# JavierMtz5/robotic_manipulator_rloa

Measured on AMD Instinct MI355X. Metric: env-steps/s (= learn() updates/s at update_freq=1,num_updates=1), KUKA 6-DoF NAF batch=256, higher is better.
Workload: dtype f32; 1 GPU; configs[1]: kuka shapes S=21 A=6 H=256, 64 envs/GPU, batch 256, HBM replay 1000000, HIP NAF head (hadamard P), 64 learn() per vector step; launch=hipGraph, parallelism=single, chain=rows, fused_kernels=bb,ep,gb,hk,s2, grad_exchange=none

## Files before the change

### include/naf_hip.h

```cpp
#ifndef NAF_HIP_H
#define NAF_HIP_H

#include <stddef.h>
#include <stdint.h>

#ifdef __cplusplus
extern "C" {
#endif

#define NAF_OK 0
#define NAF_ERR_ARG (-1)
#define NAF_ERR_STATE (-2)

#define NAF_P_HADAMARD 0
#define NAF_P_MATMUL 1

#define NAF_ACTION_TRUNC_INT 0
#define NAF_ACTION_FLOAT 1

typedef struct naf_replay naf_replay_t;

#define NAF_XGMI_MAX_WORLD 8
#define NAF_XGMI_HANDLE_BYTES 64
typedef struct {
// ... 11 lines not shown
int naf_timeline_read(int kernel_id, long long* out);

int naf_host_store_supported(int device);
int naf_host_publish(void* dst_device, const void* src_host, size_t bytes);
int naf_host_publish_launch(void* dst_device, const void* src_host, size_t bytes, void* graph_exec, void* stream);
int naf_host_store_alloc(size_t bytes, void** out_device_ptr);
int naf_host_store_free(void* device_ptr);
int naf_host_store_selftest(void* dst_device, int n_patterns, void* stream);

int naf_replay_row_floats(int S, int A);
int naf_replay_row_off_next_state(int S, int A);
int naf_replay_create(uint64_t capacity, int S, int A, float* rows, uint64_t* meta, naf_replay_t** out);
int naf_replay_destroy(naf_replay_t* h);
int naf_replay_size(naf_replay_t* h, uint64_t* size_out , void* stream);
int naf_replay_add_batch(naf_replay_t* h, const float* src_rows, int n, void* stream);
int naf_replay_add_counted(naf_replay_t* h, const float* src_rows, const int32_t* n_word, int n_max, void* stream);
int naf_replay_sample_indices(naf_replay_t* h, uint64_t seed, const uint64_t* counter_dev, uint64_t counter_off,
                              int32_t* idx, int B, int n_batches, int without_replacement, void* stream);
int naf_replay_sample_scratch_ints(int B);
int naf_replay_sample_indices_big(naf_replay_t* h, uint64_t seed, const uint64_t* counter_dev, uint64_t counter_off, int32_t* idx,
                                  int B, int n_batches, int without_replacement, int32_t* scratch, void* stream);
int naf_replay_batch_row_floats(int S, int A);
int naf_replay_gather_rows(naf_replay_t* h, const int32_t* idx, float* out_rows, int n, int out_ld, int action_mode,
                           void* stream);
int naf_replay_gather_soa(naf_replay_t* h, const int32_t* idx, float* s, float* u, float* r, float* s2,
                          float* d, int n, int action_mode, void* stream);
int naf_counter_add(uint64_t* p, uint64_t inc, void* stream);

int naf_head_fwd(const float* heads_pre, int ldh, const float* u, int ldu, float* q, float* mu_out ,
                 int B, int A, int p_mode, void* stream);
// ... 164 lines not shown
int naf_adam_polyak_fused(float* theta, const float* g, float* m, float* v, float* theta_target,
                          const float* partials, int n_partials, float max_norm, float lr, float beta1, float beta2,
                          float eps, float tau, float one_minus_tau, const int32_t* step_dev, float inv_world, size_t n,
                          void* stream);
int naf_polyak_update(float* target, const float* main, float tau, float one_minus_tau, size_t n, void* stream);

#define NAF_STEP_SPEC_INTS 12
typedef struct naf_step_copies {
    const void* src[3];
    void* dst[3];
    int n_words[3];
} naf_step_copies_t;
int naf_step_prep(naf_replay_t* h, const float* src_row, const int32_t* n_word, float* row_out, uint64_t seed,
                  uint64_t* counter_dev, int32_t* idx_out, float* out_rows, int out_ld, int action_mode, float* mom, int B,
                  int without_replacement, int32_t* spec_rec, const int32_t* idx_spec, const naf_step_copies_t* copies, void* stream);
typedef struct naf_step_prefetch {
    naf_replay_t* replay;
    uint64_t seed;
    uint64_t* counter_dev;
    int32_t* idx_spec;
    float* out_rows;
    int out_ld, action_mode;
    float* mom;
    int B, without_replacement;
    int32_t* spec_rec;
    int mode;
    const float* src_row;
    const int32_t* n_word;
    float* row_out;
    int32_t* idx_out;
// ... 40 lines not shown
                               uint64_t* host_errors, uint32_t* host_seq, uint32_t* action_rec, const naf_step_prefetch_t* prefetch,
                               int obs_system_scope, const naf_bb_layer1_t* layer1, void* stream);

typedef struct naf_episode_record {
    double score;
    int32_t frames;
    int32_t done;
    float last_reward;
    int32_t episode;
    uint32_t step_lo;
    uint32_t env;
} naf_episode_record_t;
int naf_synth_env_step(float* env_state, const float* actions, float* out_rows, float* obs_next, int E, int A,
                       uint64_t seed, const uint64_t* counter_dev, int max_frames, naf_episode_record_t* records,
                       int record_slots, void* stream);
#define NAF_SYNTH_PRESET_FLOATS 23
int naf_synth_env_reset(float* env_state, float* obs, int E, int A, uint64_t seed, uint64_t counter,
                        const float* preset_host, int preset_floats, void* stream);
int naf_synth_env_state_floats(int A);

#define NAF_CHAIN_BLOB_VERSION 1
#define NAF_CHAIN_HEADER_FLOATS 16
#define NAF_CHAIN_JOINT_FLOATS 24
#define NAF_CHAIN_SEGMENT_FLOATS 8
#define NAF_CHAIN_SCENE_FLOATS 8
#define NAF_CHAIN_ERR_VERSION (-11)
#define NAF_CHAIN_ERR_SIZE (-12)
#define NAF_CHAIN_ERR_COUNTS (-13)
#define NAF_CHAIN_ERR_VALUE (-14)
#define NAF_CHAIN_ERR_EE (-15)
// ... 61 lines not shown
```

### robotic_manipulator_rloa_amd/_lib.py

```python
from __future__ import annotations

import ctypes as C
import os
import re
import shutil
import subprocess
from typing import Optional

CSRC = os.path.join(os.path.dirname(os.path.abspath(__file__)), "csrc")
LIB_PATH = os.path.join(CSRC, "libnaf_hip.so")
SOURCES = ["lib.hip", "replay.hip", "naf_head.hip", "bn_relu.hip", "fused_layers.hip", "big_batch.hip", "gemm_bundle.hip", "optim.hip",
           "synth_env.hip", "xgmi_reduce.hip", "policy_act.hip", "step_path.hip", "naf_head_wide.hip",
           "state_digest.hip", "chain_env.hip"]
HEADERS = ["common.h", "head_body.h", "bn_tile.h", "xgmi_dev.h", "adam_body.h", "bn2bwd_fold.h", "act_body.h", "moments_body.h", "sample_body.h", "replay_dev.h", os.path.join("..", "..", "include", "naf_hip.h")]

P_HADAMARD, P_MATMUL = 0, 1
ACTION_TRUNC_INT, ACTION_FLOAT = 0, 1
NORM_CHUNK = 4096


class NafHipError(RuntimeError):
    pass


# ... 117 lines not shown
_vp, _i, _f, _u64, _sz, _i64 = C.c_void_p, C.c_int, C.c_float, C.c_uint64, C.c_size_t, C.c_int64

_PROTOS = {
    "naf_hip_abi_version": [],
    "naf_hip_arch": [],
    "naf_timeline_read": [_i, _vp],
    "naf_host_store_supported": [_i],
    "naf_host_publish": [_vp, _vp, _sz],
    "naf_host_publish_launch": [_vp, _vp, _sz, _vp, _vp],
    "naf_replay_row_floats": [_i, _i],
    "naf_replay_row_off_next_state": [_i, _i],
    "naf_replay_create": [_u64, _i, _i, _vp, _vp, C.POINTER(_vp)],
    "naf_replay_destroy": [_vp],
    "naf_replay_size": [_vp, C.POINTER(_u64), _vp],
    "naf_replay_add_batch": [_vp, _vp, _i, _vp],
    "naf_replay_add_counted": [_vp, _vp, _vp, _i, _vp],
    "naf_replay_sample_indices": [_vp, _u64, _vp, _u64, _vp, _i, _i, _i, _vp],
    "naf_replay_sample_scratch_ints": [_i],
    "naf_replay_sample_indices_big": [_vp, _u64, _vp, _u64, _vp, _i, _i, _i, _vp, _vp],
    "naf_replay_batch_row_floats": [_i, _i],
    "naf_replay_gather_rows": [_vp, _vp, _vp, _i, _i, _i, _vp],
    "naf_replay_gather_soa": [_vp, _vp, _vp, _vp, _vp, _vp, _vp, _i, _i, _vp],
    "naf_counter_add": [_vp, _u64, _vp],
    "naf_head_fwd": [_vp, _i, _vp, _i, _vp, _vp, _i, _i, _i, _vp],
    "naf_head_bwd": [_vp, _i, _vp, _i, _vp, _vp, _i, _i, _i, _vp],
    "naf_head_fwd_bwd_mse": [_vp, _i, _vp, _i, _vp, _i, _vp, _i, _f, _vp, _vp, _vp, _i, _i, _i, _vp],
    "naf_head_fwd_bwd_mse_splitk": [_vp, _i64, _vp, _i, _i, _vp, _i, _vp, _i, _f, _vp, _vp, _vp, _i, _i, _i, _vp],
    "naf_act_noise": [_vp, _i, _vp, _u64, _vp, _u64, _f, _i, _i, _i, _vp],
    "naf_bn_relu_fwd_train": [_vp, _i64, _i, _vp, _vp, _vp, _i64, _vp, _vp, _i64, _vp, _i64, _i, _vp, _vp, _i, _i, _i,
                              _f, _f, _vp],
# ... 15 lines not shown
                           _f, _f, _vp, _vp],
    "naf_bb_linear_stats_adam": [_vp, _i64, _i, _vp, _vp, _i64, _vp, _i64, _i, _vp, _i, _i, _i, _i, _vp, _vp],
    "naf_bb_layer2_head_rows": [_i],
    "naf_bb_layer2_head_exchange_floats": [_i, _i],
    "naf_bb_layer2_head": [_vp, _i64, _i, _vp, _vp, _i64, _vp, _vp, _vp, _i64, _vp, _i, _vp, _vp, _vp, _i64, _i, _i, _vp, _i, _vp,
                           _i, _f, _vp, _vp, _vp, _vp, _i, _vp, _i, _i, _i, _i, _f, _f, _vp, _vp],
    "naf_bb_layer1_bwd_kp": [_i],
    "naf_bb_layer1_bwd_finish_blocks": [_i],
    "naf_bb_layer1_bwd_finish": [_vp, _i, _vp, _i, _vp, _i, _vp, _vp, _vp, _vp, _vp, _vp, _vp, _vp, _vp, _vp, _vp, _vp, _vp, _i, _i,
                                 _vp, _i, _vp, _vp, _vp, _sz, _vp],
    "naf_gemm_bundle": [_vp, _i, _vp],
    "naf_grad_norm_partials": [_vp, _sz, _vp, _vp, _vp],
    "naf_adam_polyak_fused": [_vp, _vp, _vp, _vp, _vp, _vp, _i, _f, _f, _f, _f, _f, _f, _f, _vp, _f, _sz, _vp],
    "naf_polyak_update": [_vp, _vp, _f, _f, _sz, _vp],
    "naf_synth_env_step": [_vp, _vp, _vp, _vp, _i, _i, _u64, _vp, _i, _vp, _i, _vp],
    "naf_synth_env_reset": [_vp, _vp, _i, _i, _u64, _u64, _vp, _i, _vp],
    "naf_synth_env_state_floats": [_i],
    "naf_policy_act": [_vp, _i, _i, _vp, _vp, _vp, _vp, _vp, _vp, _vp, _vp, _vp, _i, _i, _vp, _vp, _vp, _vp, _f, _i, _vp, _i,
                       _vp, _u64, _vp, _vp, _f, _i, _i, _i, _vp],
    "naf_step_prep": [_vp, _vp, _vp, _vp, _u64, _vp, _vp, _vp, _i, _i, _vp, _i, _i, _vp, _vp, _vp, _vp],
    "naf_adam_polyak_act_sync_ints": [],
    "naf_host_store_alloc": [_sz, C.POINTER(_vp)],
    "naf_host_store_free": [_vp],
    "naf_host_store_selftest": [_vp, _i, _vp],
    "naf_step_prefetch": [_vp, _vp],
    "naf_step_launch": [_vp, _vp, _sz, _vp, _vp, _vp, _vp, C.c_int],
    "naf_adam_polyak_act": [_vp, _vp, _vp, _vp, _vp, _u64, _vp, _f, _i, _vp, _vp, _vp, _vp, _vp, _i, _vp],
    "naf_adam_polyak_act_layer1": [_vp, _vp, _vp, _vp, _vp, _u64, _vp, _f, _i, _vp, _vp, _vp, _vp, _vp, _i, _vp, _vp],
    "naf_xgmi_chunk_floats": [],
    "naf_xgmi_create": [_i, _i, _sz, C.c_double, C.POINTER(_vp)],
    "naf_xgmi_set_timeout": [_vp, C.c_double],
    "naf_xgmi_mem_kind": [_vp],
    "naf_xgmi_export": [_vp, _vp],
    "naf_xgmi_connect": [_vp, _vp, _vp],
    "naf_xgmi_connect_local": [_vp, _vp],
# ... 152 lines not shown
```

### robotic_manipulator_rloa_amd/csrc/replay.hip

```cpp
#include <stdlib.h>
#include "common.h"
#include "sample_body.h"
#include "replay_dev.h"
#include "../../include/naf_hip.h"
#include <new>

extern "C" int naf_replay_row_floats(int S, int A) {
    if (S <= 0 || A <= 0) return NAF_ERR_ARG;
    int need = naf_row_off_done(S, A) + 1;
    int rf = 32;
    while (rf < need) rf *= 2;
    return rf;
}

extern "C" int naf_replay_row_off_next_state(int S, int A) {
    if (S <= 0 || A <= 0) return NAF_ERR_ARG;
    return naf_row_off_s2(S, A);
}

extern "C" int naf_replay_create(uint64_t capacity, int S, int A, float* rows, uint64_t* meta, naf_replay_t** out) {
    if (!out || !rows || !meta || capacity == 0 || S <= 0 || A <= 0 || A > NAF_MAX_A_WIDE) return NAF_ERR_ARG;
    if (capacity > 0x7fffffffull) return NAF_ERR_ARG;
    if (((uintptr_t)rows & 15) != 0) return NAF_ERR_ARG;
    naf_replay* h = new (std::nothrow) naf_replay;
// ... 25 lines not shown
}

__global__ void replay_add_rows_kernel(float4* __restrict__ ring, const uint64_t* __restrict__ meta,
                                       const float4* __restrict__ src, int n, uint64_t cap, int rf4_shift) {
    const uint64_t head = meta[META_HEAD];
    const int rf4 = 1 << rf4_shift;
    for (int64_t g = (int64_t)blockIdx.x * blockDim.x + threadIdx.x; g < ((int64_t)n << rf4_shift);
         g += (int64_t)gridDim.x * blockDim.x) {
        int64_t r = g >> rf4_shift;
        int c = (int)(g & (rf4 - 1));
        uint64_t phys = (head + (uint64_t)r) % cap;
        ring[(phys << rf4_shift) + c] = src[g];
    }
}

__global__ void replay_advance_kernel(uint64_t* meta, uint64_t n, uint64_t cap) {
    if (blockIdx.x == 0 && threadIdx.x == 0) {
        uint64_t head = meta[META_HEAD], size = meta[META_SIZE];
        meta[META_HEAD] = (head + n) % cap;
        size += n;
        meta[META_SIZE] = size > cap ? cap : size;
        meta[META_TOTAL] += n;
    }
}

__global__ __launch_bounds__(1024) void replay_add_small_kernel(float4* __restrict__ ring, uint64_t* meta,
                                                                const float4* __restrict__ src, int n,
                                                                uint64_t cap, int rf4_shift) {
    const uint64_t head = meta[META_HEAD];
    const uint64_t size = meta[META_SIZE];
    const int rf4 = 1 << rf4_shift;
    __syncthreads();
    int g = threadIdx.x;
    if (g < (n << rf4_shift)) {
        int r = g >> rf4_shift;
        int c = g & (rf4 - 1);
        uint64_t phys = (head + (uint64_t)r) % cap;
        ring[(phys << rf4_shift) + c] = src[g];
    }
    if (threadIdx.x == 0) {
        meta[META_HEAD] = (head + (uint64_t)n) % cap;
        uint64_t s2 = size + (uint64_t)n;
        meta[META_SIZE] = s2 > cap ? cap : s2;
        meta[META_TOTAL] += (uint64_t)n;
    }
}

__global__ __launch_bounds__(1024) void replay_add_counted_kernel(float4* __restrict__ ring, uint64_t* meta,
                                                                  const float4* __restrict__ src, const int32_t* n_word,
                                                                  int n_max, uint64_t cap, int rf4_shift) {
    int n = __builtin_nontemporal_load(n_word);
    n = n < 0 ? 0 : (n > n_max ? n_max : n);
    const uint64_t head = meta[META_HEAD];
    const uint64_t size = meta[META_SIZE];
    const int rf4 = 1 << rf4_shift;
    __syncthreads();
    int g = threadIdx.x;
    if (g < (n << rf4_shift)) {
        int r = g >> rf4_shift;
// ... 3 lines not shown
    }
    if (threadIdx.x == 0 && n > 0) {
        meta[META_HEAD] = (head + (uint64_t)n) % cap;
        uint64_t s2 = size + (uint64_t)n;
        meta[META_SIZE] = s2 > cap ? cap : s2;
        meta[META_TOTAL] += (uint64_t)n;
    }
}

static inline int ilog2_exact(int x) {
    int s = 0;
    while ((1 << s) < x) ++s;
    return s;
}

extern "C" int naf_replay_add_batch(naf_replay_t* h, const float* src_rows, int n, void* stream) {
    if (!h || h->magic != NAF_REPLAY_MAGIC) return NAF_ERR_STATE;
    if (!src_rows || n < 0 || (uint64_t)n > h->capacity || ((uintptr_t)src_rows & 15) != 0) return NAF_ERR_ARG;
    if (n == 0) return NAF_OK;
    hipStream_t st = (hipStream_t)stream;
    const int rf4 = h->row_floats / 4;
    const int sh = ilog2_exact(rf4);
    if ((int64_t)n * rf4 <= 1024) {
        int threads = naf_round_up(n * rf4, 64);
        replay_add_small_kernel<<<1, threads, 0, st>>>((float4*)h->rows, h->meta, (const float4*)src_rows, n,
                                                        h->capacity, sh);
        NAF_CHECK_LAUNCH();
        return NAF_OK;
    }
    int64_t total = (int64_t)n * rf4;
    int blocks = (int)((total + 255) / 256);
    if (blocks > 4096) blocks = 4096;
    replay_add_rows_kernel<<<blocks, 256, 0, st>>>((float4*)h->rows, h->meta, (const float4*)src_rows, n,
                                                    h->capacity, sh);
    NAF_CHECK_LAUNCH();
    replay_advance_kernel<<<1, 64, 0, st>>>(h->meta, (uint64_t)n, h->capacity);
    NAF_CHECK_LAUNCH();
    return NAF_OK;
}

extern "C" int naf_replay_add_counted(naf_replay_t* h, const float* src_rows, const int32_t* n_word, int n_max, void* stream) {
    if (!h || h->magic != NAF_REPLAY_MAGIC) return NAF_ERR_STATE;
    const int rf4 = h->row_floats / 4;
    if (!src_rows || !n_word || n_max < 1 || (uint64_t)n_max > h->capacity || (int64_t)n_max * rf4 > 1024 ||
        ((uintptr_t)src_rows & 15) != 0 || ((uintptr_t)n_word & 3) != 0)
        return NAF_ERR_ARG;
    replay_add_counted_kernel<<<1, naf_round_up(n_max * rf4, 64), 0, (hipStream_t)stream>>>(
        (float4*)h->rows, h->meta, (const float4*)src_rows, n_word, n_max, h->capacity, ilog2_exact(rf4));
    NAF_CHECK_LAUNCH();
    return NAF_OK;
}

__global__ __launch_bounds__(1024) void replay_sample_kernel(const uint64_t* __restrict__ meta, uint64_t seed,
// ... 312 lines not shown
```

### robotic_manipulator_rloa_amd/csrc/replay_dev.h

```cpp
#pragma once
#include "common.h"
#include "../../include/naf_hip.h"

struct naf_replay {
    uint64_t capacity;
    int S, A, row_floats;
    float* rows;
    uint64_t* meta;
    uint32_t magic;
};
#define NAF_REPLAY_MAGIC 0x4e414652u

enum { META_HEAD = 0, META_SIZE = 1, META_TOTAL = 2, META_SAMPLE_CTR = 3, META_BAD_IDX = 7 };
```

### robotic_manipulator_rloa_amd/csrc/step_path.hip

```cpp
#include <string.h>
#include "common.h"
#include "../../include/naf_hip.h"
NAF_TL_DECL(g_tl_sp);
#ifdef NAF_TIMELINE
#define BM_MARK(slot) NAF_TL(g_tl_sp, NAF_TL_STEP_PREP, slot)
#define SB_MARK(slot) NAF_TL(g_tl_sp, NAF_TL_STEP_PREP, slot)
#endif
#include "act_body.h"
#include "adam_body.h"
#include "head_body.h"
#ifdef NAF_TIMELINE
#define BB_L1_TL(slot, is_first, is_last) NAF_TL_FL(g_tl_sp, NAF_TL_BB_LAYER1, slot, is_first, is_last)
#define BB_L1_TL_T(slot, is_first, is_last, thread) NAF_TL_FL_T(g_tl_sp, NAF_TL_BB_LAYER1, slot, is_first, is_last, thread)
#endif
#include "layer1_body.h"
#include "moments_body.h"
#include "replay_dev.h"
#include "sample_body.h"

NAF_TL_READER(naf_tl_read_sp, g_tl_sp)

#define SP_THREADS 1024
#define SP_RPT 4
#define SP_CACHE_ROWS 256
// ... 392 lines not shown
        for (const void* k : ks) {
            hipError_t e = hipFuncSetAttribute(k, hipFuncAttributeMaxDynamicSharedMemorySize, SP_MAX_DYN_LDS);
            if (e != hipSuccess) return (int)e;
        }
        raised_dev[dev] = 1;
    }
    const bool cache = sp_cached(B, out_ld);
    if (k4 <= 6 && cache) step_prep_kernel<6, true><<<1, SP_THREADS, lds, (hipStream_t)stream>>>(P);
    else if (k4 <= 6) step_prep_kernel<6, false><<<1, SP_THREADS, lds, (hipStream_t)stream>>>(P);
    else if (cache) step_prep_kernel<8, true><<<1, SP_THREADS, lds, (hipStream_t)stream>>>(P);
    else step_prep_kernel<8, false><<<1, SP_THREADS, lds, (hipStream_t)stream>>>(P);
    NAF_CHECK_LAUNCH();
    return NAF_OK;
}

#define AA_THREADS 512
#define AA_H 256
#define AA_L1_WGS 8
#define AA_L1_ROWS (AA_H / AA_L1_WGS)
#define AA_L2_WGS 32
#define AA_SYNC_RIDE (16 + 4 * 2 * AA_H)
#define AA_POLL_TICKS 200000LL

typedef float aa_f4 __attribute__((ext_vector_type(4)));

struct AdamActArgs {
    AdamArgs ad;
    int64_t off_W1, off_b1, off_g1, off_be1, off_W2, off_b2, off_g2, off_be2, off_Wh;
    int S, NH, NHP, HP, A;
    const float* obs;
// ... 745 lines not shown
```

### robotic_manipulator_rloa_amd/csrc/synth_env.hip

```cpp
#include "common.h"
#include "../../include/naf_hip.h"

#define ENV_STATE_FLOATS 36
#define ENV_OFF_VAR 24
#define ENV_OFF_SCORE 32
#define ENV_DT (1.0f / 240.0f)

struct EnvCfg {
    float link[8];
};
__constant__ EnvCfg c_env = {{0.34f, 0.02f, 0.40f, 0.02f, 0.40f, 0.13f, 0.05f, 0.05f}};

__device__ static inline void fk_chain(const float* q, int A, float* ee, const float* obstacle, float obstacle_r,
                                       bool* hit) {
    float R[9] = {1, 0, 0, 0, 1, 0, 0, 0, 1};
    float p[3] = {0.f, 0.f, 0.f};
    bool h = false;
    for (int k = 0; k < A; ++k) {
        float c = cosf(q[k]), s = sinf(q[k]);
        float N[9];
        if ((k & 1) == 0) {
            for (int r = 0; r < 3; ++r) {
                N[r * 3 + 0] = R[r * 3 + 0] * c + R[r * 3 + 1] * s;
                N[r * 3 + 1] = -R[r * 3 + 0] * s + R[r * 3 + 1] * c;
// ... 45 lines not shown
    for (int k = 0; k < 8; ++k) { st[14 + k] = preset.v[k]; st[ENV_OFF_VAR + k] = preset.v[15 + k]; }
    st[34] = st[35] = 0.f;
    for (int k = 0; k < 3; ++k) { st[8 + k] = preset.v[8 + k]; st[11 + k] = preset.v[11 + k]; }
    if (preset.v[14] > 0.f) {
        Philox4 p = philox4x32_10((uint32_t)seed, (uint32_t)(seed >> 32), (uint32_t)e, 0x4f425354u, 0x9E3779B9u, 0x243F6A88u);
        for (int k = 0; k < 3; ++k) st[11 + k] += (naf_u01(p.v[k]) * 2.f - 1.f) * preset.v[14];
    }
    st[23] = 0.f;
    env_reset_one(st, e, A, seed, ctr);
    float qd[8] = {0, 0, 0, 0, 0, 0, 0, 0}, ee[3];
    bool hit;
    fk_chain(st, A, ee, st + 11, 0.06f, &hit);
    write_obs(obs + (int64_t)e * (2 * A + 9), st, qd, ee, st + 8, st + 11, A);
}

__global__ void synth_env_step_kernel(float* env_state, const float* __restrict__ actions, float* __restrict__ out_rows,
                                      float* __restrict__ obs_next, int E, int A, int row_floats, uint64_t seed,
                                      const uint64_t* counter_dev, int max_frames, naf_episode_record_t* __restrict__ records,
                                      int record_slots) {
    int e = blockIdx.x * blockDim.x + threadIdx.x;
    if (e >= E) return;
    const int S = 2 * A + 9;
    float* st = env_state + (int64_t)e * ENV_STATE_FLOATS;
    float* row = out_rows + (int64_t)e * row_floats;
    float* ob = obs_next + (int64_t)e * S;
    const uint64_t ctr = counter_dev ? *counter_dev : 0ull;

    for (int k = 0; k < S; ++k) row[k] = ob[k];
    float a[8], ee[3];
    for (int k = 0; k < A; ++k) {
        a[k] = actions[(int64_t)e * A + k];
        row[S + k] = a[k];
        st[k] += ENV_DT * a[k];
    }
    bool hit;
    fk_chain(st, A, ee, st + 11, 0.06f, &hit);
    float dx = ee[0] - st[8], dy = ee[1] - st[9], dz = ee[2] - st[10];
    float dist = sqrtf(dx * dx + dy * dy + dz * dz);
    const bool reached = dist < 0.05f;
    float reward = reached ? 250.f : (hit ? -1000.f : -(dist - 0.05f));
    float done = (reached || hit) ? 1.f : 0.f;
    const int off_s2 = naf_row_off_s2(S, A), off_d = naf_row_off_done(S, A);
    row[S + A] = reward;
    for (int k = S + A + 1; k < off_s2; ++k) row[k] = 0.f;
    write_obs(row + off_s2, st, a, ee, st + 8, st + 11, A);
    row[off_d] = done;
// ... 13 lines not shown
        rec.step_lo = (uint32_t)ctr;
        rec.env = (uint32_t)e;
        records[(int64_t)(ctr % (uint64_t)record_slots) * E + e] = rec;
    }
    if (over) {
        st[23] += 1.f;
        env_reset_one(st, e, A, seed, ctr * 0x9E3779B97F4A7C15ull + (uint64_t)st[23]);
        float qd0[8] = {0, 0, 0, 0, 0, 0, 0, 0};
        fk_chain(st, A, ee, st + 11, 0.06f, &hit);
        write_obs(ob, st, qd0, ee, st + 8, st + 11, A);
    } else {
        for (int k = 0; k < S; ++k) ob[k] = row[off_s2 + k];
    }
}

extern "C" int naf_synth_env_state_floats(int A) { return (A > 0 && A <= NAF_MAX_A) ? ENV_STATE_FLOATS : NAF_ERR_ARG; }

extern "C" int naf_synth_env_reset(float* env_state, float* obs, int E, int A, uint64_t seed, uint64_t counter,
                                   const float* preset_host, int preset_floats, void* stream) {
    if (!env_state || !obs || E <= 0 || A <= 0 || A > NAF_MAX_A) return NAF_ERR_ARG;
    if (preset_host && preset_floats != 15 && preset_floats != NAF_SYNTH_PRESET_FLOATS) return NAF_ERR_ARG;
    EnvPreset p = {{0.9f, 0.45f, 0.f, 0.f, 0.f, 0.f, 0.f, 0.f, 0.4f, 0.85f, 0.71f, 0.45f, 0.55f, 0.55f, 0.f,
                    0.1f, 0.1f, 0.1f, 0.1f, 0.1f, 0.1f, 0.1f, 0.1f}};
    if (preset_host)
        for (int k = 0; k < preset_floats; ++k) p.v[k] = preset_host[k];
    synth_env_reset_kernel<<<(E + 63) / 64, 64, 0, (hipStream_t)stream>>>(env_state, obs, E, A, seed, counter, p);
    NAF_CHECK_LAUNCH();
    return NAF_OK;
}

extern "C" int naf_synth_env_step(float* env_state, const float* actions, float* out_rows, float* obs_next, int E, int A,
                                  uint64_t seed, const uint64_t* counter_dev, int max_frames, naf_episode_record_t* records,
                                  int record_slots, void* stream) {
    if (!env_state || !actions || !out_rows || !obs_next || E <= 0 || A <= 0 || A > NAF_MAX_A) return NAF_ERR_ARG;
    if (records && (record_slots <= 0 || !counter_dev)) return NAF_ERR_ARG;
    int rf = naf_replay_row_floats(2 * A + 9, A);
    synth_env_step_kernel<<<(E + 63) / 64, 64, 0, (hipStream_t)stream>>>(env_state, actions, out_rows, obs_next, E, A, rf,
                                                                         seed, counter_dev, max_frames, records, record_slots);
    NAF_CHECK_LAUNCH();
    return NAF_OK;
}
```

### robotic_manipulator_rloa_amd/engine.py

```python
from __future__ import annotations

import json
import os
from dataclasses import dataclass
from typing import Callable, Dict, List, Optional, Tuple

import numpy as np
import torch

from . import _lib
from ._lib import check, ptr, stream_ptr
from .learner import ActPath, Learner
from .presets import ROBOT_PRESETS, device_env_preset
from .utils.replay_buffer import ReplayBuffer


class _StateSnapshot:

    def __init__(self, learner: Learner, replay: Optional[ReplayBuffer], extra=()):
        self.pairs = [(t, t.clone()) for t in (learner.theta2, learner.grad, learner.adam_m, learner.adam_v,
                                               learner.bn_stats, learner.step_dev, learner.partials)]
        if replay is not None and replay._handle is not None:
            self.pairs += [(t, t.clone()) for t in (replay.meta, replay._sample_ctr)]
        self.pairs += [(t, t.clone()) for t in extra]
# ... 13 lines not shown
    torch.cuda.synchronize()
    snapshot.restore()
    if after_warmup is not None:
        after_warmup()
    g = torch.cuda.CUDAGraph()
    with torch.cuda.graph(g):
        body()
    snapshot.restore()
    torch.cuda.synchronize()
    return g


class UpdateChunk:

    def __init__(self, learner: Learner, replay: ReplayBuffer, n_updates: int, teacher_forced: bool = False,
                 use_graph: bool = True, gather_outside_graph: bool = False):
        self.L, self.replay, self.U = learner, replay, int(n_updates)
        self.teacher_forced = teacher_forced
        self.gather_outside_graph = gather_outside_graph
        self.gather_events = None
        self.empty_events = None
        B, dev = learner.B, learner.dev
        if replay.batch_size != B:
            raise ValueError("ReplayBuffer.batch_size must equal the learner's batch size")
        self.idx = torch.zeros(self.U, B, dtype=torch.int32, device=dev)
        brf = learner.lay.batch_row_floats
        self._batch_store = torch.zeros(self.U * B * brf + 64, dtype=torch.float32, device=dev)
        self.batch = self._batch_store[:self.U * B * brf].view(self.U, B, brf)
        self.loss_parts = torch.zeros(self.U, learner.n_loss_wg, dtype=torch.float32, device=dev)
        self.moments = (torch.zeros(self.U, 2, learner.mom_floats, dtype=torch.float32, device=dev)
                        if "bb" in learner.fuse else None)
        self.graph: Optional[torch.cuda.CUDAGraph] = None
        self.use_graph = use_graph

    def _sample_gather(self) -> None:
        if not self.teacher_forced:
            self.replay.sample_indices(self.idx, self.U)
        ev = self.gather_events
        if ev is not None:
            ev[0].record()
        self.replay.gather_rows(self.idx, self.batch, self.U * self.L.B)
        if ev is not None:
            ev[1].record()
            if self.empty_events is not None:
                self.empty_events[0].record()
                self.empty_events[1].record()

    def _updates(self, moments_ready: bool = False, defer_last: bool = False) -> None:
        if self.moments is not None and not moments_ready:
            self.L.moments(self.batch.view(self.U * self.L.B, -1), self.moments, self.U)
        d = self.L.defer_ok
        for k in range(self.U):
            self.L.learn_rows(self.batch[k], self.loss_parts[k], None if self.moments is None else self.moments[k],
                              pending=d and k > 0, defer=d and (k < self.U - 1 or defer_last))

    def _body(self) -> None:
        self._sample_gather()
        self._updates()

    def _snapshot(self, extra=()) -> _StateSnapshot:
        return _StateSnapshot(self.L, self.replay, (self.idx, self.batch, self.loss_parts) + tuple(extra))

    def capture(self) -> None:
        self.replay.flush()
        snap = self._snapshot()
        if self.gather_outside_graph:
            self._sample_gather()
            self.graph = _capture(self._updates, snap)
        else:
            self.graph = _capture(self._body, snap)

# ... 515 lines not shown

    def finish(self) -> Dict[int, Tuple[float, int]]:
        if self.write:
            torch.save(self._state_dict_fn(), self.model_path)
        return self.scores


class DeviceEnvLoop:

    PRESETS = {name: device_env_preset(name) for name in ROBOT_PRESETS}

    def __init__(self, learner: Learner, replay: Optional[ReplayBuffer], n_envs: int, seed: int, max_frames: int = 400,
                 noise_scale: float = 1.0, use_graph: bool = True, robot: str = "kuka", obstacle_jitter: float = 0.0,
                 preset: Optional[List[float]] = None, variation: Optional[List[float]] = None, records: bool = False,
                 drain_every: int = 64, chain=None, target=None, obstacle=None, obstacle_radius: float = 0.06,
                 target_range=None, obstacle_range=None, scene_margin: float = 0.02):
        self.L, self.replay, self.E = learner, replay, int(n_envs)
        lay, dev = learner.lay, learner.dev
        self.lib = learner.lib
        self.seed = int(seed) & 0xFFFFFFFFFFFFFFFF
        self.max_frames = int(max_frames)
        self.noise_scale = float(noise_scale)
        self.actor = ActPath(learner, self.E, seed=self.seed ^ 0xA5A5A5A5)
        self.chain, self._chain_env = chain, None
        import ctypes
        if chain is not None:
            self._open_chain(chain, target, obstacle, obstacle_radius, obstacle_jitter, target_range, obstacle_range, scene_margin)
            nst = self.lib.naf_chain_env_state_floats(self._chain_env)
        elif target_range is not None or obstacle_range is not None:
            raise ValueError("DeviceEnvLoop: target_range / obstacle_range belong to a chain model's scene")
        elif lay.A > 8:
# ... 10 lines not shown
        base = list(preset) if preset is not None else list(self.PRESETS[robot])
        if len(base) != 14:
            raise ValueError("DeviceEnvLoop: preset = [initial joint positions(8) | target xyz | obstacle xyz]")
        var = [0.1] * 8 if variation is None else ([float(v) for v in variation] + [0.0] * 8)[:8]
        self._preset = (ctypes.c_float * 23)(*(base + [float(obstacle_jitter)] + var))
        self.drain_every = max(1, int(drain_every))
        self.records = None
        self._finished: List[tuple] = []
        self._steps = 0
        self._copied = 0
        self._inflight = None
        if records:
            self.records = torch.zeros(self.drain_every, self.E, 8, dtype=torch.int32, device=dev)
            self._pins = [torch.zeros(self.drain_every, self.E, 8, dtype=torch.int32).pin_memory() for _ in range(2)]
            self._pin_i = 0
        self.reset()

    def _open_chain(self, chain, target, obstacle, obstacle_radius, obstacle_jitter, target_range=None, obstacle_range=None,
                    scene_margin=0.02) -> None:
        import ctypes
        lay = self.L.lay
        if chain.A != lay.A or chain.state_size != lay.S:
            raise ValueError(f"DeviceEnvLoop: the chain model drives {chain.A} joints (state size {chain.state_size}), the agent "
                             f"was built for action_size {lay.A} / state_size {lay.S}")
        if target is None or obstacle is None or len(target) != 3 or len(obstacle) != 3:
            raise ValueError("DeviceEnvLoop(chain=...): give target and obstacle as xyz")
        blob = np.ascontiguousarray(chain.pack(), np.float32)
        handle = ctypes.c_void_p()
        check(self.lib.naf_chain_env_create(blob.ctypes.data, int(blob.size), ctypes.byref(handle)), "chain_env_create")
        self._chain_env = handle
# ... 22 lines not shown
            check(self.lib.naf_synth_env_reset(ptr(self.env_state), ptr(self.actor.obs), self.E, self.L.lay.A, self.seed, 0,
                                               self._preset, 23, stream_ptr()), "synth_env_reset")
        self.step_ctr.zero_()
        self._steps = self._copied = 0
        self._inflight = None
        self._finished = []

    def _body(self) -> None:
        st = stream_ptr()
        self.actor.act(self.noise_scale)
        slots = self.drain_every if self.records is not None else 0
        if self._chain_env is not None:
            check(self.lib.naf_chain_env_step(self._chain_env, ptr(self.env_state), ptr(self.actor.actions), ptr(self.rows),
                                              ptr(self.actor.obs), self.E, self.seed, ptr(self.step_ctr), self.max_frames,
                                              ptr(self.records), slots, st), "chain_env_step")
        else:
            check(self.lib.naf_synth_env_step(ptr(self.env_state), ptr(self.actor.actions), ptr(self.rows),
                                              ptr(self.actor.obs), self.E, self.L.lay.A, self.seed, ptr(self.step_ctr),
                                              self.max_frames, ptr(self.records), slots, st), "synth_env_step")
        check(self.lib.naf_counter_add(ptr(self.step_ctr), 1, st), "counter_add")
        if self.replay is not None:
            check(self.lib.naf_replay_add_batch(self.replay.handle, ptr(self.rows), self.E, st), "replay_add_batch")

    def capture(self) -> None:
        warmup = 2
        extra = (self.env_state, self.rows, self.step_ctr, self.actor.obs, self.actor.counter, self.actor.actions)
        if self.records is not None:
            extra += (self.records,)
        snap = _StateSnapshot(self.L, self.replay, extra)
        put_back = None
        if self.replay is not None:
            head = int(self.replay.meta[0].item())
            pos = (head + torch.arange(warmup * self.E, device=self.L.dev)) % self.replay.buffer_size
            saved = self.replay.rows[pos].clone()
# ... 169 lines not shown
```

### robotic_manipulator_rloa_amd/utils/replay_buffer.py

```python
from __future__ import annotations

import random
from typing import Optional, Tuple

import numpy as np
import torch

from .. import _lib
from .._lib import check, ptr, stream_ptr

_DIRECT_ROWS = 16
_STAGE_ROWS = 1024


class ReplayBuffer:

    def __init__(self, buffer_size: int, batch_size: int, device, seed: int, state_size: Optional[int] = None,
                 action_size: Optional[int] = None, action_mode: int = _lib.ACTION_TRUNC_INT,
                 without_replacement: bool = True):
        _lib.require_gpu()
        self.lib = _lib.load()
        self.device = torch.device(device)
        self.buffer_size = int(buffer_size)
        self.batch_size = int(batch_size)
# ... 103 lines not shown
        if self.batch_size > 4096:
            per = self.lib.naf_replay_sample_scratch_ints(self.batch_size)
            if per < 0:
                raise ValueError(f"batch_size {self.batch_size}: the replay sampler draws minibatches of at most 1,048,576")
            if self._sample_scratch is None or self._sample_scratch.numel() < per * int(n_batches):
                self._sample_scratch = torch.zeros(per * int(n_batches), dtype=torch.int32, device=self.device)
            check(self.lib.naf_replay_sample_indices_big(self.handle, self.seed, ptr(self._sample_ctr), 0, ptr(idx_out),
                                                         self.batch_size, int(n_batches), int(self.without_replacement),
                                                         ptr(self._sample_scratch), stream_ptr()), "naf_replay_sample_indices_big")
        else:
            check(self.lib.naf_replay_sample_indices(self.handle, self.seed, ptr(self._sample_ctr), 0, ptr(idx_out),
                                                     self.batch_size, int(n_batches), int(self.without_replacement),
                                                     stream_ptr()), "naf_replay_sample_indices")
        check(self.lib.naf_counter_add(ptr(self._sample_ctr), int(n_batches), stream_ptr()), "naf_counter_add")

    def gather_rows(self, idx: torch.Tensor, out_rows: torch.Tensor, n: int) -> None:
        self._join_side()
        if not out_rows.is_contiguous() or out_rows.numel() < int(n) * out_rows.shape[-1]:
            raise ValueError("gather_rows: out_rows must be contiguous and hold n rows")
        check(self.lib.naf_replay_gather_rows(self.handle, ptr(idx), ptr(out_rows), int(n), int(out_rows.shape[-1]),
                                              self.action_mode, stream_ptr()), "naf_replay_gather_rows")

    def sample(self, idx: Optional[torch.Tensor] = None) -> Tuple[torch.Tensor, ...]:
        self._join_side()
        self.flush()
        B, dev = self.batch_size, self.device
        if idx is None and len(self) < B:
            raise ValueError("Sample larger than population or is negative")
        if idx is None:
            self.sample_indices(self._idx, 1)
# ... 27 lines not shown
```

Before: 35020 env-steps/s.

## Fuse replay sample/gather/moments and env step with replay append into single launches

Adds a single kernel that samples indices, gathers and truncates replay rows into LDS, computes batch-norm moments and advances the sample counter with a last-block ticket. This replaces the separate sample, counter-add, gather and moments launches in each update chunk. It also adds a fused synthetic env step that writes rows straight into the replay ring and bumps the step counter, and folds the counter increment into replay add for the chain env path. The fused paths are enabled by default when shapes fit, at the cost of more complex kernels and a new meta ticket word.

```diff
diff --git a/include/naf_hip.h b/include/naf_hip.h
--- a/include/naf_hip.h
+++ b/include/naf_hip.h
@@ -49,6 +49,7 @@
 int naf_replay_destroy(naf_replay_t* h);
 int naf_replay_size(naf_replay_t* h, uint64_t* size_out , void* stream);
 int naf_replay_add_batch(naf_replay_t* h, const float* src_rows, int n, void* stream);
+int naf_replay_add_batch_ctr(naf_replay_t* h, const float* src_rows, int n, uint64_t* ctr, void* stream);
 int naf_replay_add_counted(naf_replay_t* h, const float* src_rows, const int32_t* n_word, int n_max, void* stream);
 int naf_replay_sample_indices(naf_replay_t* h, uint64_t seed, const uint64_t* counter_dev, uint64_t counter_off,
                               int32_t* idx, int B, int n_batches, int without_replacement, void* stream);
@@ -243,6 +244,9 @@
 int naf_step_prep(naf_replay_t* h, const float* src_row, const int32_t* n_word, float* row_out, uint64_t seed,
                   uint64_t* counter_dev, int32_t* idx_out, float* out_rows, int out_ld, int action_mode, float* mom, int B,
                   int without_replacement, int32_t* spec_rec, const int32_t* idx_spec, const naf_step_copies_t* copies, void* stream);
+int naf_replay_prep_chunk_fits(int S, int A, int B);
+int naf_replay_prep_chunk(naf_replay_t* h, uint64_t seed, uint64_t* counter_dev, int32_t* idx, float* out_rows, int out_ld,
+                          int action_mode, float* mom, int B, int n_batches, int without_replacement, void* stream);
 typedef struct naf_step_prefetch {
     naf_replay_t* replay;
     uint64_t seed;
@@ -313,6 +317,9 @@
 int naf_synth_env_step(float* env_state, const float* actions, float* out_rows, float* obs_next, int E, int A,
                        uint64_t seed, const uint64_t* counter_dev, int max_frames, naf_episode_record_t* records,
                        int record_slots, void* stream);
+int naf_synth_env_step_append(float* env_state, const float* actions, float* out_rows, float* obs_next, int E, int A,
+                              uint64_t seed, uint64_t* counter_dev, int max_frames, naf_episode_record_t* records,
+                              int record_slots, naf_replay_t* h, void* stream);
 #define NAF_SYNTH_PRESET_FLOATS 23
 int naf_synth_env_reset(float* env_state, float* obs, int E, int A, uint64_t seed, uint64_t counter,
                         const float* preset_host, int preset_floats, void* stream);
diff --git a/robotic_manipulator_rloa_amd/_lib.py b/robotic_manipulator_rloa_amd/_lib.py
--- a/robotic_manipulator_rloa_amd/_lib.py
+++ b/robotic_manipulator_rloa_amd/_lib.py
@@ -155,6 +155,7 @@
     "naf_replay_destroy": [_vp],
     "naf_replay_size": [_vp, C.POINTER(_u64), _vp],
     "naf_replay_add_batch": [_vp, _vp, _i, _vp],
+    "naf_replay_add_batch_ctr": [_vp, _vp, _i, _vp, _vp],
     "naf_replay_add_counted": [_vp, _vp, _vp, _i, _vp],
     "naf_replay_sample_indices": [_vp, _u64, _vp, _u64, _vp, _i, _i, _i, _vp],
     "naf_replay_sample_scratch_ints": [_i],
@@ -200,11 +201,14 @@
     "naf_adam_polyak_fused": [_vp, _vp, _vp, _vp, _vp, _vp, _i, _f, _f, _f, _f, _f, _f, _f, _vp, _f, _sz, _vp],
     "naf_polyak_update": [_vp, _vp, _f, _f, _sz, _vp],
     "naf_synth_env_step": [_vp, _vp, _vp, _vp, _i, _i, _u64, _vp, _i, _vp, _i, _vp],
+    "naf_synth_env_step_append": [_vp, _vp, _vp, _vp, _i, _i, _u64, _vp, _i, _vp, _i, _vp, _vp],
     "naf_synth_env_reset": [_vp, _vp, _i, _i, _u64, _u64, _vp, _i, _vp],
     "naf_synth_env_state_floats": [_i],
     "naf_policy_act": [_vp, _i, _i, _vp, _vp, _vp, _vp, _vp, _vp, _vp, _vp, _vp, _i, _i, _vp, _vp, _vp, _vp, _f, _i, _vp, _i,
                        _vp, _u64, _vp, _vp, _f, _i, _i, _i, _vp],
     "naf_step_prep": [_vp, _vp, _vp, _vp, _u64, _vp, _vp, _vp, _i, _i, _vp, _i, _i, _vp, _vp, _vp, _vp],
+    "naf_replay_prep_chunk_fits": [_i, _i, _i],
+    "naf_replay_prep_chunk": [_vp, _u64, _vp, _vp, _vp, _i, _i, _vp, _i, _i, _i, _vp],
     "naf_adam_polyak_act_sync_ints": [],
     "naf_host_store_alloc": [_sz, C.POINTER(_vp)],
     "naf_host_store_free": [_vp],
diff --git a/robotic_manipulator_rloa_amd/csrc/replay.hip b/robotic_manipulator_rloa_amd/csrc/replay.hip
--- a/robotic_manipulator_rloa_amd/csrc/replay.hip
+++ b/robotic_manipulator_rloa_amd/csrc/replay.hip
@@ -63,8 +63,9 @@
     }
 }
 
-__global__ void replay_advance_kernel(uint64_t* meta, uint64_t n, uint64_t cap) {
+__global__ void replay_advance_kernel(uint64_t* meta, uint64_t n, uint64_t cap, uint64_t* ctr) {
     if (blockIdx.x == 0 && threadIdx.x == 0) {
+        if (ctr) *ctr += 1;
         uint64_t head = meta[META_HEAD], size = meta[META_SIZE];
         meta[META_HEAD] = (head + n) % cap;
         size += n;
@@ -75,7 +76,7 @@
 
 __global__ __launch_bounds__(1024) void replay_add_small_kernel(float4* __restrict__ ring, uint64_t* meta,
                                                                 const float4* __restrict__ src, int n,
-                                                                uint64_t cap, int rf4_shift) {
+                                                                uint64_t cap, int rf4_shift, uint64_t* ctr) {
     const uint64_t head = meta[META_HEAD];
     const uint64_t size = meta[META_SIZE];
     const int rf4 = 1 << rf4_shift;
@@ -92,6 +93,7 @@
         uint64_t s2 = size + (uint64_t)n;
         meta[META_SIZE] = s2 > cap ? cap : s2;
         meta[META_TOTAL] += (uint64_t)n;
+        if (ctr) *ctr += 1;
     }
 }
 
@@ -125,17 +127,17 @@
     return s;
 }
 
-extern "C" int naf_replay_add_batch(naf_replay_t* h, const float* src_rows, int n, void* stream) {
+static int replay_add_batch(naf_replay_t* h, const float* src_rows, int n, uint64_t* ctr, void* stream) {
     if (!h || h->magic != NAF_REPLAY_MAGIC) return NAF_ERR_STATE;
     if (!src_rows || n < 0 || (uint64_t)n > h->capacity || ((uintptr_t)src_rows & 15) != 0) return NAF_ERR_ARG;
-    if (n == 0) return NAF_OK;
+    if (n == 0) return ctr ? naf_counter_add(ctr, 1, stream) : NAF_OK;
     hipStream_t st = (hipStream_t)stream;
     const int rf4 = h->row_floats / 4;
     const int sh = ilog2_exact(rf4);
     if ((int64_t)n * rf4 <= 1024) {
         int threads = naf_round_up(n * rf4, 64);
         replay_add_small_kernel<<<1, threads, 0, st>>>((float4*)h->rows, h->meta, (const float4*)src_rows, n,
-                                                        h->capacity, sh);
+                                                        h->capacity, sh, ctr);
         NAF_CHECK_LAUNCH();
         return NAF_OK;
     }
@@ -145,9 +147,18 @@
     replay_add_rows_kernel<<<blocks, 256, 0, st>>>((float4*)h->rows, h->meta, (const float4*)src_rows, n,
                                                     h->capacity, sh);
     NAF_CHECK_LAUNCH();
-    replay_advance_kernel<<<1, 64, 0, st>>>(h->meta, (uint64_t)n, h->capacity);
-    NAF_CHECK_LAUNCH();
-    return NAF_OK;
+    replay_advance_kernel<<<1, 64, 0, st>>>(h->meta, (uint64_t)n, h->capacity, ctr);
+    NAF_CHECK_LAUNCH();
+    return NAF_OK;
+}
+
+extern "C" int naf_replay_add_batch(naf_replay_t* h, const float* src_rows, int n, void* stream) {
+    return replay_add_batch(h, src_rows, n, nullptr, stream);
+}
+
+extern "C" int naf_replay_add_batch_ctr(naf_replay_t* h, const float* src_rows, int n, uint64_t* ctr, void* stream) {
+    if (!ctr) return NAF_ERR_ARG;
+    return replay_add_batch(h, src_rows, n, ctr, stream);
 }
 
 extern "C" int naf_replay_add_counted(naf_replay_t* h, const float* src_rows, const int32_t* n_word, int n_max, void* stream) {
diff --git a/robotic_manipulator_rloa_amd/csrc/replay_dev.h b/robotic_manipulator_rloa_amd/csrc/replay_dev.h
--- a/robotic_manipulator_rloa_amd/csrc/replay_dev.h
+++ b/robotic_manipulator_rloa_amd/csrc/replay_dev.h
@@ -11,4 +11,4 @@
 };
 #define NAF_REPLAY_MAGIC 0x4e414652u
 
-enum { META_HEAD = 0, META_SIZE = 1, META_TOTAL = 2, META_SAMPLE_CTR = 3, META_BAD_IDX = 7 };
+enum { META_HEAD = 0, META_SIZE = 1, META_TOTAL = 2, META_SAMPLE_CTR = 3, META_TICKET = 4, META_BAD_IDX = 7 };
diff --git a/robotic_manipulator_rloa_amd/csrc/step_path.hip b/robotic_manipulator_rloa_amd/csrc/step_path.hip
--- a/robotic_manipulator_rloa_amd/csrc/step_path.hip
+++ b/robotic_manipulator_rloa_amd/csrc/step_path.hip
@@ -430,6 +430,151 @@
     return NAF_OK;
 }
 
+struct PrepChunkArgs {
+    const float4* ring;
+    uint64_t* meta;
+    uint64_t cap;
+    int rf4_shift;
+    uint64_t seed;
+    uint64_t* counter;
+    int32_t* idx;
+    float4* out_rows;
+    float* mom;
+    int w4, trunc_lo, trunc_hi, off_s2_4;
+    int B, without_replacement, hash_bits;
+};
+
+template <int K4>
+__global__ __launch_bounds__(SP_THREADS) void replay_prep_chunk_kernel(const PrepChunkArgs P) {
+    extern __shared__ __attribute__((aligned(16))) unsigned char sp_smem[];
+    constexpr int KP = 4 * K4, REC = KP + KP * KP;
+    BmShared* S = (BmShared*)sp_smem;
+    int* sPos = (int*)(sp_smem + 2 * sizeof(BmShared));
+    float4* sRows = (float4*)(sp_smem + 2 * sizeof(BmShared) + (size_t)naf_round_up(P.B, 4) * sizeof(int));
+    int* vals = (int*)sp_smem;
+    const int tid = threadIdx.x, B = P.B, u = blockIdx.x;
+    const uint64_t head = P.meta[META_HEAD], size = P.meta[META_SIZE];
+    const uint64_t ctr0 = *P.counter;
+
+    replay_sample_body(vals, tid, SP_THREADS, size, ctr0 + (uint64_t)u, P.seed, B, P.without_replacement, P.hash_bits);
+    const uint64_t base = head + P.cap - size;
+    int myidx[4];
+#pragma unroll
+    for (int k = 0; k < 4; ++k) {
+        const int t = tid + SP_THREADS * k;
+        int64_t i = t < B ? (int64_t)vals[t] : 0;
+        myidx[k] = (int)i;
+        const bool bad = i < 0 || (uint64_t)i >= size;
+        if (bad && t < B) atomicAdd((unsigned long long*)&P.meta[META_BAD_IDX], 1ull);
+        if (bad) i = 0;
+        uint64_t pos = base + (uint64_t)i;
+        pos = pos >= P.cap ? pos - P.cap : pos;
+        pos = pos >= P.cap ? pos - P.cap : pos;
+        if (t < B) sPos[t] = (int)pos;
+    }
+    __syncthreads();
+
+    const unsigned w4 = (unsigned)P.w4;
+    const int total4 = B * P.w4;
+    for (int j0 = tid; j0 < total4; j0 += SP_THREADS * SP_RPT) {
+        float4 v[SP_RPT];
+        int col[SP_RPT];
+#pragma unroll
+        for (int k = 0; k < SP_RPT; ++k) {
+            const int j = j0 + SP_THREADS * k;
+            const unsigned jj = j < total4 ? (unsigned)j : 0u;
+            const unsigned r = jj / w4;
+            col[k] = (int)(jj - r * w4);
+            v[k] = P.ring[((int64_t)sPos[r] << P.rf4_shift) + col[k]];
+        }
+#pragma unroll
+        for (int k = 0; k < SP_RPT; ++k) {
+            const int j = j0 + SP_THREADS * k;
+            if (j < total4) sRows[j] = sp_trunc(v[k], 4 * col[k], P.trunc_lo, P.trunc_hi);
+        }
+    }
+
+    const int net = tid >> 9;
+    const int c0 = net ? P.off_s2_4 : 0;
+    bb_moments_body<K4>([&](int row, int q) { return sRows[row * P.w4 + c0 + q]; }, S[net], tid & (BM_THREADS - 1),
+                        P.mom + ((int64_t)u * 2 + net) * REC, B);
+    float4* const out = P.out_rows + (int64_t)u * total4;
+    for (int j = tid; j < total4; j += SP_THREADS) out[j] = sRows[j];
+#pragma unroll
+    for (int k = 0; k < 4; ++k) {
+        const int t = tid + SP_THREADS * k;
+        if (t < B) P.idx[(int64_t)u * B + t] = myidx[k];
+    }
+    if (tid == 0) {
+        unsigned* ticket = (unsigned*)&P.meta[META_TICKET];
+        const unsigned n = gridDim.x;
+        if (__hip_atomic_fetch_add(ticket, 1u, __ATOMIC_RELAXED, __HIP_MEMORY_SCOPE_AGENT) == n - 1u) {
+            __hip_atomic_store(ticket, 0u, __ATOMIC_RELAXED, __HIP_MEMORY_SCOPE_AGENT);
+            *P.counter = ctr0 + (uint64_t)n;
+        }
+    }
+}
+
+static size_t prep_chunk_lds(int B, int out_ld) {
+    const int bits = sample_hash_bits(B);
+    if (B <= 0 || B > 4096 || sample_lds_ints(B, bits) * sizeof(int) > 2 * sizeof(BmShared)) return 0;
+    return 2 * sizeof(BmShared) + (size_t)naf_round_up(B, 4) * sizeof(int) + (size_t)B * out_ld * sizeof(float);
+}
+
+extern "C" int naf_replay_prep_chunk_fits(int S, int A, int B) {
+    if (S <= 0 || A <= 0 || (S + 3) / 4 > 8) return 0;
+    const int out_ld = naf_replay_batch_row_floats(S, A), k4d = (S + 3) / 4 <= 6 ? 6 : 8;
+    if (naf_replay_row_floats(S, A) > 4 * SP_MAX_RF4 || naf_row_off_s2(S, A) + 4 * k4d > out_ld) return 0;
+    const size_t lds = prep_chunk_lds(B, out_ld);
+    return lds != 0 && lds <= SP_MAX_DYN_LDS;
+}
+
+extern "C" int naf_replay_prep_chunk(naf_replay_t* h, uint64_t seed, uint64_t* counter_dev, int32_t* idx, float* out_rows, int out_ld,
+                                     int action_mode, float* mom, int B, int n_batches, int without_replacement, void* stream) {
+    if (!h || h->magic != NAF_REPLAY_MAGIC) return NAF_ERR_STATE;
+    if (!counter_dev || !idx || !out_rows || !mom || n_batches <= 0 || (((uintptr_t)out_rows | (uintptr_t)mom) & 15) != 0)
+        return NAF_ERR_ARG;
+    if (action_mode != NAF_ACTION_TRUNC_INT && action_mode != NAF_ACTION_FLOAT) return NAF_ERR_ARG;
+    if (out_ld != naf_replay_batch_row_floats(h->S, h->A) || naf_replay_prep_chunk_fits(h->S, h->A, B) != 1) return NAF_ERR_ARG;
+    if ((int64_t)n_batches * B * (out_ld / 4) >= 0x7fffffffll) return NAF_ERR_ARG;
+    PrepChunkArgs P;
+    P.ring = (const float4*)h->rows;
+    P.meta = h->meta;
+    P.cap = h->capacity;
+    int sh = 0;
+    while ((1 << sh) < h->row_floats / 4) ++sh;
+    P.rf4_shift = sh;
+    P.seed = seed;
+    P.counter = counter_dev;
+    P.idx = idx;
+    P.out_rows = (float4*)out_rows;
+    P.mom = mom;
+    P.w4 = out_ld / 4;
+    P.trunc_lo = h->S;
+    P.trunc_hi = h->S + h->A;
+    if (action_mode == NAF_ACTION_FLOAT) P.trunc_lo = P.trunc_hi = 0x7fffffff;
+    P.off_s2_4 = naf_row_off_s2(h->S, h->A) / 4;
+    P.B = B;
+    P.without_replacement = without_replacement;
+    P.hash_bits = sample_hash_bits(B);
+    const size_t lds = prep_chunk_lds(B, out_ld);
+    static int raised_dev[64];
+    int dev = 0;
+    if (hipGetDevice(&dev) != hipSuccess || dev < 0 || dev >= 64) dev = 0;
+    if (!raised_dev[dev]) {
+        const void* ks[2] = {(const void*)replay_prep_chunk_kernel<6>, (const void*)replay_prep_chunk_kernel<8>};
+        for (const void* k : ks) {
+            hipError_t e = hipFuncSetAttribute(k, hipFuncAttributeMaxDynamicSharedMemorySize, SP_MAX_DYN_LDS);
+            if (e != hipSuccess) return (int)e;
+        }
+        raised_dev[dev] = 1;
+    }
+    if ((h->S + 3) / 4 <= 6) replay_prep_chunk_kernel<6><<<n_batches, SP_THREADS, lds, (hipStream_t)stream>>>(P);
+    else replay_prep_chunk_kernel<8><<<n_batches, SP_THREADS, lds, (hipStream_t)stream>>>(P);
+    NAF_CHECK_LAUNCH();
+    return NAF_OK;
+}
+
 #define AA_THREADS 512
 #define AA_H 256
 #define AA_L1_WGS 8
diff --git a/robotic_manipulator_rloa_amd/csrc/synth_env.hip b/robotic_manipulator_rloa_amd/csrc/synth_env.hip
--- a/robotic_manipulator_rloa_amd/csrc/synth_env.hip
+++ b/robotic_manipulator_rloa_amd/csrc/synth_env.hip
@@ -1,4 +1,5 @@
 #include "common.h"
+#include "replay_dev.h"
 #include "../../include/naf_hip.h"
 
 #define ENV_STATE_FLOATS 36
@@ -83,22 +84,14 @@
     write_obs(obs + (int64_t)e * (2 * A + 9), st, qd, ee, st + 8, st + 11, A);
 }
 
-__global__ void synth_env_step_kernel(float* env_state, const float* __restrict__ actions, float* __restrict__ out_rows,
-                                      float* __restrict__ obs_next, int E, int A, int row_floats, uint64_t seed,
-                                      const uint64_t* counter_dev, int max_frames, naf_episode_record_t* __restrict__ records,
-                                      int record_slots) {
-    int e = blockIdx.x * blockDim.x + threadIdx.x;
-    if (e >= E) return;
+__device__ __forceinline__ static void env_step_one(float* st, float* row, float* ob, const float* act, int e, int E, int A,
+                                                    int row_floats, uint64_t seed, uint64_t ctr, int max_frames,
+                                                    naf_episode_record_t* __restrict__ records, int record_slots) {
     const int S = 2 * A + 9;
-    float* st = env_state + (int64_t)e * ENV_STATE_FLOATS;
-    float* row = out_rows + (int64_t)e * row_floats;
-    float* ob = obs_next + (int64_t)e * S;
-    const uint64_t ctr = counter_dev ? *counter_dev : 0ull;
-
     for (int k = 0; k < S; ++k) row[k] = ob[k];
     float a[8], ee[3];
     for (int k = 0; k < A; ++k) {
-        a[k] = actions[(int64_t)e * A + k];
+        a[k] = act[k];
         row[S + k] = a[k];
         st[k] += ENV_DT * a[k];
     }
@@ -142,6 +135,62 @@
     }
 }
 
+__global__ void synth_env_step_kernel(float* env_state, const float* __restrict__ actions, float* __restrict__ out_rows,
+                                      float* __restrict__ obs_next, int E, int A, int row_floats, uint64_t seed,
+                                      const uint64_t* counter_dev, int max_frames, naf_episode_record_t* __restrict__ records,
+                                      int record_slots) {
+    int e = blockIdx.x * blockDim.x + threadIdx.x;
+    if (e >= E) return;
+    const int S = 2 * A + 9;
+    const uint64_t ctr = counter_dev ? *counter_dev : 0ull;
+    env_step_one(env_state + (int64_t)e * ENV_STATE_FLOATS, out_rows + (int64_t)e * row_floats, obs_next + (int64_t)e * S,
+                 actions + (int64_t)e * A, e, E, A, row_floats, seed, ctr, max_frames, records, record_slots);
+}
+
+#define ENV_ST_LD 38
+__global__ __launch_bounds__(1024) void synth_env_step_append_kernel(float* env_state, const float* __restrict__ actions,
+                                                                     float4* __restrict__ out_rows, float* obs_next,
+                                                                     float4* __restrict__ ring, uint64_t* meta, uint64_t cap,
+                                                                     int rf4_shift, int E, int A, uint64_t seed,
+                                                                     uint64_t* counter_dev, int max_frames,
+                                                                     naf_episode_record_t* __restrict__ records, int record_slots) {
+    extern __shared__ __attribute__((aligned(16))) float env_smem[];
+    const int S = 2 * A + 9, rf4 = 1 << rf4_shift, rf = 4 * rf4, rld = rf + 1;
+    float* sSt = env_smem;
+    float* sRow = sSt + E * ENV_ST_LD;
+    float* sOb = sRow + E * rld;
+    float* sAct = sOb + E * S;
+    const int tid = threadIdx.x, nt = blockDim.x;
+    const uint64_t ctr = *counter_dev;
+    const uint64_t head = meta[META_HEAD];
+    const uint64_t size = meta[META_SIZE];
+    for (int i = tid; i < E * ENV_STATE_FLOATS; i += nt) sSt[(i / ENV_STATE_FLOATS) * ENV_ST_LD + i % ENV_STATE_FLOATS] = env_state[i];
+    for (int i = tid; i < E * S; i += nt) sOb[i] = obs_next[i];
+    for (int i = tid; i < E * A; i += nt) sAct[i] = actions[i];
+    __syncthreads();
+    if (tid < E)
+        env_step_one(sSt + tid * ENV_ST_LD, sRow + tid * rld, sOb + tid * S, sAct + tid * A, tid, E, A, rf, seed, ctr, max_frames,
+                     records, record_slots);
+    __syncthreads();
+    if (tid < (E << rf4_shift)) {
+        const int r = tid >> rf4_shift, c = tid & (rf4 - 1);
+        const float* p = sRow + r * rld + 4 * c;
+        const float4 v = make_float4(p[0], p[1], p[2], p[3]);
+        const uint64_t phys = (head + (uint64_t)r) % cap;
+        out_rows[tid] = v;
+        ring[(phys << rf4_shift) + c] = v;
+    }
+    for (int i = tid; i < E * ENV_STATE_FLOATS; i += nt) env_state[i] = sSt[(i / ENV_STATE_FLOATS) * ENV_ST_LD + i % ENV_STATE_FLOATS];
+    for (int i = tid; i < E * S; i += nt) obs_next[i] = sOb[i];
+    if (tid == 0) {
+        meta[META_HEAD] = (head + (uint64_t)E) % cap;
+        const uint64_t s2 = size + (uint64_t)E;
+        meta[META_SIZE] = s2 > cap ? cap : s2;
+        meta[META_TOTAL] += (uint64_t)E;
+        *counter_dev = ctr + 1;
+    }
+}
+
 extern "C" int naf_synth_env_state_floats(int A) { return (A > 0 && A <= NAF_MAX_A) ? ENV_STATE_FLOATS : NAF_ERR_ARG; }
 
 extern "C" int naf_synth_env_reset(float* env_state, float* obs, int E, int A, uint64_t seed, uint64_t counter,
@@ -168,3 +217,23 @@
     NAF_CHECK_LAUNCH();
     return NAF_OK;
 }
+
+extern "C" int naf_synth_env_step_append(float* env_state, const float* actions, float* out_rows, float* obs_next, int E, int A,
+                                         uint64_t seed, uint64_t* counter_dev, int max_frames, naf_episode_record_t* records,
+                                         int record_slots, naf_replay_t* h, void* stream) {
+    if (!h || h->magic != NAF_REPLAY_MAGIC) return NAF_ERR_STATE;
+    if (!env_state || !actions || !out_rows || !obs_next || !counter_dev || E <= 0 || A <= 0 || A > NAF_MAX_A) return NAF_ERR_ARG;
+    if (records && record_slots <= 0) return NAF_ERR_ARG;
+    const int S = 2 * A + 9, rf = naf_replay_row_floats(S, A), rf4 = rf / 4;
+    if (h->S != S || h->A != A || h->row_floats != rf || (uint64_t)E > h->capacity || (int64_t)E * rf4 > 1024 ||
+        ((uintptr_t)out_rows & 15) != 0)
+        return NAF_ERR_ARG;
+    int sh = 0;
+    while ((1 << sh) < rf4) ++sh;
+    const size_t lds = (size_t)E * (ENV_ST_LD + rf + 1 + S + A) * sizeof(float);
+    synth_env_step_append_kernel<<<1, naf_round_up(E * rf4, 64), lds, (hipStream_t)stream>>>(
+        env_state, actions, (float4*)out_rows, obs_next, (float4*)h->rows, h->meta, h->capacity, sh, E, A, seed, counter_dev,
+        max_frames, records, record_slots);
+    NAF_CHECK_LAUNCH();
+    return NAF_OK;
+}
diff --git a/robotic_manipulator_rloa_amd/engine.py b/robotic_manipulator_rloa_amd/engine.py
--- a/robotic_manipulator_rloa_amd/engine.py
+++ b/robotic_manipulator_rloa_amd/engine.py
@@ -51,7 +51,7 @@
 class UpdateChunk:
 
     def __init__(self, learner: Learner, replay: ReplayBuffer, n_updates: int, teacher_forced: bool = False,
-                 use_graph: bool = True, gather_outside_graph: bool = False):
+                 use_graph: bool = True, gather_outside_graph: bool = False, fused_prep: Optional[bool] = None):
         self.L, self.replay, self.U = learner, replay, int(n_updates)
         self.teacher_forced = teacher_forced
         self.gather_outside_graph = gather_outside_graph
@@ -69,6 +69,11 @@
                         if "bb" in learner.fuse else None)
         self.graph: Optional[torch.cuda.CUDAGraph] = None
         self.use_graph = use_graph
+        fits = (self.moments is not None and not teacher_forced and not gather_outside_graph and replay._handle is not None and
+                replay.prep_chunk_fits())
+        if fused_prep and not fits:
+            raise ValueError("UpdateChunk(fused_prep=True): this shape or mode takes the four launches (ReplayBuffer.prep_chunk_fits)")
+        self.one_launch_prep = fits if fused_prep is None else bool(fused_prep)
 
     def _sample_gather(self) -> None:
         if not self.teacher_forced:
@@ -92,6 +97,10 @@
                               pending=d and k > 0, defer=d and (k < self.U - 1 or defer_last))
 
     def _body(self) -> None:
+        if self.one_launch_prep and self.gather_events is None:
+            self.replay.prep_chunk(self.idx, self.batch, self.moments, self.U)
+            self._updates(moments_ready=True)
+            return
         self._sample_gather()
         self._updates()
 
@@ -637,7 +646,7 @@
                  noise_scale: float = 1.0, use_graph: bool = True, robot: str = "kuka", obstacle_jitter: float = 0.0,
                  preset: Optional[List[float]] = None, variation: Optional[List[float]] = None, records: bool = False,
                  drain_every: int = 64, chain=None, target=None, obstacle=None, obstacle_radius: float = 0.06,
-                 target_range=None, obstacle_range=None, scene_margin: float = 0.02):
+                 target_range=None, obstacle_range=None, scene_margin: float = 0.02, fused_step: Optional[bool] = None):
         self.L, self.replay, self.E = learner, replay, int(n_envs)
         lay, dev = learner.lay, learner.dev
         self.lib = learner.lib
@@ -678,6 +687,12 @@
             self.records = torch.zeros(self.drain_every, self.E, 8, dtype=torch.int32, device=dev)
             self._pins = [torch.zeros(self.drain_every, self.E, 8, dtype=torch.int32).pin_memory() for _ in range(2)]
             self._pin_i = 0
+        fits = (replay is not None and chain is None and self.E * (lay.row_floats // 4) <= 1024 and self.E <= replay.buffer_size and
+                (replay.S, replay.A) == (2 * lay.A + 9, lay.A))
+        if fused_step and not fits:
+            raise ValueError("DeviceEnvLoop(fused_step=True): needs the stand-in env, a replay and E * row_floats / 4 <= 1024")
+        self.fused_step = fits if fused_step is None else bool(fused_step)
+        self._fold_ctr = fused_step is not False and chain is not None and replay is not None
         self.reset()
 
     def _open_chain(self, chain, target, obstacle, obstacle_radius, obstacle_jitter, target_range=None, obstacle_range=None,
@@ -730,10 +745,20 @@
             check(self.lib.naf_chain_env_step(self._chain_env, ptr(self.env_state), ptr(self.actor.actions), ptr(self.rows),
                                               ptr(self.actor.obs), self.E, self.seed, ptr(self.step_ctr), self.max_frames,
                                               ptr(self.records), slots, st), "chain_env_step")
+        elif self.fused_step:
+            check(self.lib.naf_synth_env_step_append(ptr(self.env_state), ptr(self.actor.actions), ptr(self.rows),
+                                                     ptr(self.actor.obs), self.E, self.L.lay.A, self.seed, ptr(self.step_ctr),
+                                                     self.max_frames, ptr(self.records), slots, self.replay.handle, st),
+                  "synth_env_step_append")
+            return
         else:
             check(self.lib.naf_synth_env_step(ptr(self.env_state), ptr(self.actor.actions), ptr(self.rows),
                                               ptr(self.actor.obs), self.E, self.L.lay.A, self.seed, ptr(self.step_ctr),
                                               self.max_frames, ptr(self.records), slots, st), "synth_env_step")
+        if self._fold_ctr:
+            check(self.lib.naf_replay_add_batch_ctr(self.replay.handle, ptr(self.rows), self.E, ptr(self.step_ctr), st),
+                  "replay_add_batch_ctr")
+            return
         check(self.lib.naf_counter_add(ptr(self.step_ctr), 1, st), "counter_add")
         if self.replay is not None:
             check(self.lib.naf_replay_add_batch(self.replay.handle, ptr(self.rows), self.E, st), "replay_add_batch")
diff --git a/robotic_manipulator_rloa_amd/utils/replay_buffer.py b/robotic_manipulator_rloa_amd/utils/replay_buffer.py
--- a/robotic_manipulator_rloa_amd/utils/replay_buffer.py
+++ b/robotic_manipulator_rloa_amd/utils/replay_buffer.py
@@ -141,6 +141,16 @@
                                                      stream_ptr()), "naf_replay_sample_indices")
         check(self.lib.naf_counter_add(ptr(self._sample_ctr), int(n_batches), stream_ptr()), "naf_counter_add")
 
+    def prep_chunk_fits(self) -> bool:
+        return self.S is not None and self.lib.naf_replay_prep_chunk_fits(self.S, self.A, self.batch_size) == 1
+
+    def prep_chunk(self, idx_out: torch.Tensor, out_rows: torch.Tensor, moments: torch.Tensor, n_batches: int) -> None:
+        self._join_side()
+        self._gen += 1
+        check(self.lib.naf_replay_prep_chunk(self.handle, self.seed, ptr(self._sample_ctr), ptr(idx_out), ptr(out_rows),
+                                             int(out_rows.shape[-1]), self.action_mode, ptr(moments), self.batch_size,
+                                             int(n_batches), int(self.without_replacement), stream_ptr()), "naf_replay_prep_chunk")
+
     def gather_rows(self, idx: torch.Tensor, out_rows: torch.Tensor, n: int) -> None:
         self._join_side()
         if not out_rows.is_contiguous() or out_rows.numel() < int(n) * out_rows.shape[-1]:
```

Result: no change. 35340 env-steps/s, median of 6 (+0.9%).
